# SunJiamei/LRP-ImageCaptioning

Measured on AMD Instinct MI355X. Metric: LRP heatmaps/sec (per predicted token) VGG16+adaptive-attn, 224x224, higher is better.
Workload: dtype bf16x3; 1 GPU; batch=32 synthetic 224x224 per GPU, VGG16 + adaptive-attention, LRP per-token heat-maps, 10 words/caption, V=10000 (BASELINE configs[1]); parallelism=image-sharded x1, RCCL weight broadcast, reverse_walk_precision=bf16x3, handles_per_gpu=2

## Files before the change

### lrp-imagecaptioning_amd/csrc/cnn_kernels.h

```cpp
#pragma once
#include <hip/hip_runtime.h>
#include "conv_igemm.h"

namespace lrp {

__device__ __forceinline__ float safe_den(float z) { return z + (z == 0.f ? 1e-7f : 0.f); }

__global__ __launch_bounds__(256) void im2col_image_kernel(const float* __restrict__ img, float* __restrict__ A1,
                                                           int NB, int H, int W) {
  const size_t idx = (size_t)blockIdx.x * 256 + threadIdx.x;
  const size_t total = (size_t)NB * H * W * 8;
  if (idx >= total) return;
  const int g = (int)(idx & 7);
  const size_t m = idx >> 3;
  const int HW = H * W;
  const int n = (int)(m / HW), rem = (int)(m - (size_t)n * HW);
  const int h = rem / W, w = rem - h * W;
  const bool neg = g >= 4;
  float v[8];
#pragma unroll
  for (int q = 0; q < 8; ++q) {
    const int kk = 8 * (g & 3) + q;
    float x = 0.f;
    if (kk < 27) {
// ... 430 lines not shown
}

__global__ __launch_bounds__(256) void top_divide_split_kernel(const float* __restrict__ R, const float* __restrict__ Ztop,
                                                               const int* __restrict__ row2img, float* __restrict__ S,
                                                               int n, size_t per_img8) {
  const size_t total = (size_t)n * per_img8;
  for (size_t i = (size_t)blockIdx.x * 256 + threadIdx.x; i < total; i += (size_t)gridDim.x * 256) {
    const int t = (int)(i / per_img8);
    const size_t e = i - (size_t)t * per_img8;
    const int img = row2img ? row2img[t] : t;
    const float* r = R + i * 8;
    const float* z = Ztop + ((size_t)img * per_img8 + e) * 8;
    float o[8];
#pragma unroll
    for (int c = 0; c < 8; ++c) o[c] = r[c] / safe_den(z[c]);
    split8_store(o, S + i * 8);
  }
}

constexpr int IMG_T_COLS = 54;
__global__ __launch_bounds__(256) void img_stencil_kernel(const float* __restrict__ T, const float* __restrict__ ximg,
                                                          const int* __restrict__ row2img, float* __restrict__ out,
                                                          int n, int H, int W, int mode) {
  const size_t total = (size_t)n * H * W;
  for (size_t i = (size_t)blockIdx.x * 256 + threadIdx.x; i < total; i += (size_t)gridDim.x * 256) {
    const int HW = H * W;
    const int t = (int)(i / HW), pix = (int)(i - (size_t)t * HW);
    const int h = pix / W, w = pix - h * W;
    float pos[3] = {0.f, 0.f, 0.f}, neg[3] = {0.f, 0.f, 0.f};
#pragma unroll
// ... 81 lines not shown
```

### lrp-imagecaptioning_amd/csrc/decoder.h

```cpp
#pragma once
#include <algorithm>
#include <functional>
#include <map>
#include <string>
#include <vector>

#include "cnn_kernels.h"
#include "common.h"
#include "conv_igemm.h"
#include "decoder_gridtd_kernels.h"
#include "decoder_batched_kernels.h"
#include "decoder_kernels.h"
#include "gradient_kernels.h"
#include "train_gemm.h"

namespace lrp {

struct StateBuf {
  DevBuf buf;
  size_t elem_bytes = 4;
};

struct Decoder {
  int kind = 0, L = 0, D = 0, H = 0, E = 0, V = 0, Tm = 0, B_max = 0, NT_max = 0, sos = 2, eos = 1;
// ... 5 lines not shown
  DevBuf xh, u, att_pre;
  DevBuf state_arena;
  std::map<std::string, StateBuf> state;
  DevBuf cap_dev;
  std::vector<int> cap_host, len_host;
  int* cap_pinned = nullptr;
  hipEvent_t ev_cap = nullptr;
  ~Decoder() {
    if (ev_cap) { (void)hipEventSynchronize(ev_cap); (void)hipEventDestroy(ev_cap); }
    if (cap_pinned) (void)hipHostFree(cap_pinned);
    if (ev_gen) { (void)hipEventSynchronize(ev_gen); (void)hipEventDestroy(ev_gen); }
    if (gen_pinned) (void)hipHostFree(gen_pinned);
  }
  int B_cur = 0;
  bool have_forward = false;
  DevBuf rctx, ravg, tailA, w_ifT_pk;
  DevBuf Wcat2, bcat2, xh1d, xh2d, zg1d, zg2d, hprojd, sprojd, h2u, rho;
  bool bx_ready = false;
  DevBuf bxWg1, bxWg2, bx_rc, bx_rh, bx_rglob, bx_q32, bx_acc32;
  DevBuf bx_g[7];
  bool grad_ready = false;
  DevBuf gW1, gW2, gWglob, gWif, g_seed, g_dc1, g_dc2, g_dg, g_out1, g_out2, g_dglob, g_dwords, g_dctx, g_davg, g_tailA;

  int init(const lrp_config& c, int64_t* total) {
    kind = c.decoder; L = c.L; D = c.D; H = c.H; E = c.E; V = c.V; Tm = c.max_caption_len;
    B_max = c.max_images; NT_max = c.max_tokens; sos = c.sos_id; eos = c.eos_id;
    if (L < 1 || D < 4 || H < 4 || E < 4 || V < 2) return fail(LRP_ERR_INVALID, "bad decoder dims");
    if (D % 8 || H % 8) return fail(LRP_ERR_UNSUPPORTED, "D and H must be multiples of 8");
    if (2 * E + 2 * H > 2048) return fail(LRP_ERR_UNSUPPORTED, "2E+2H too large for the LRP scan (bx_* / gbx_* kernels)");
    const size_t B = B_max, S = Tm + 1;
    struct Want { std::string nm; size_t bytes, eb; };
    std::vector<Want> wants;
    auto st = [&](const char* nm, size_t elems, size_t eb) -> int {
      wants.push_back({nm, elems * eb, eb});
      return LRP_OK;
    };
    if (kind == LRP_DEC_ADAPTIVE) {
      for (const char* nm : {"ht", "ct", "gt", "it_act", "ft_act", "st", "ot_act"}) LRP_TRY(st(nm, B * S * H, 4));
      LRP_TRY(st("attention", B * S * L, 4));
      LRP_TRY(st("beta", B * S, 4));
      LRP_TRY(st("context", B * S * H, 8));
      LRP_TRY(st("c_hat", B * S * H, 8));
      LRP_TRY(st("xt", B * Tm * 2 * E, 4));
      LRP_TRY(st("caption_preds", B * Tm * V, 8));
// ... 14 lines not shown
      LRP_TRY(hprojd.alloc(B * H * 8 * KS_PROJ, total));
      LRP_TRY(sprojd.alloc(B * H * 8 * KS_PROJ, total));
      LRP_TRY(st("#h2u", B * Tm * H, 8));
      LRP_TRY(rho.alloc((size_t)NT_max * Tm * H * 8, total));
    }
    LRP_TRY(vfeat.alloc(B * L * H * 4, total));
    LRP_TRY(if_pre.alloc(B * L * H * 4, total));
    if (kind == LRP_DEC_ADAPTIVE) LRP_TRY(ipre.alloc(B * L * H * 8, total));
    LRP_TRY(stat.alloc(B * L * H * 4, total));
    LRP_TRY(avg.alloc(B * D * 4, total));
    LRP_TRY(glob_pre.alloc(B * E * 4, total));
    LRP_TRY(xh.alloc(B * (2 * E + 2 * H) * 4, total));
    LRP_TRY(att_pre.alloc(B * (L + 1) * 4, total));
    LRP_TRY(st("#u", B * Tm * H, 8));
    {
      size_t off = 0;
      for (const Want& w : wants) off += (w.bytes + 255) / 256 * 256;
      LRP_TRY(state_arena.alloc(off, total));
      off = 0;
      for (const Want& w : wants) {
        if (w.nm == "#u") u.view_of(state_arena, off, w.bytes);
        else if (w.nm == "#h2u") h2u.view_of(state_arena, off, w.bytes);
        else {
          StateBuf& s = state[w.nm];
          s.elem_bytes = w.eb;
          s.buf.view_of(state_arena, off, w.bytes);
        }
        off += (w.bytes + 255) / 256 * 256;
      }
    }
    LRP_TRY(cap_dev.alloc(B * Tm * sizeof(int), total));
    LRP_TRY(rctx.alloc((size_t)NT_max * H * 8, total));
    LRP_TRY(tailA.alloc((size_t)NT_max * L * H * 4, total));
    LRP_TRY(ravg.alloc((size_t)NT_max * D * 8, total));
    cap_host.assign(B * Tm, eos);
    len_host.assign(B, 0);
    return LRP_OK;
  }

  int on_new_features(int B) {
    B_cur = B;
    have_forward = false;
    return LRP_OK;
  }
// ... 29 lines not shown
    LRP_TRY(weight_set_common(nm, ndim, shape, &n));
    DevBuf& d = raw_dev[nm];
    if (d.bytes != n * sizeof(float)) LRP_TRY(d.alloc(n * sizeof(float), total));
    LRP_HIP_CHECK(hipMemcpyAsync(d.p, data, n * sizeof(float), kind, st));
    return LRP_OK;
  }

  static void tr2d(hipStream_t st, const float* src, int lds, int rows, int cols, float* dst, int ldd) {
    hipLaunchKernelGGL(dec_transpose_kernel, dim3((cols + 31) / 32, (rows + 31) / 32), dim3(32, 8), 0, st, src, lds, rows, cols, dst, ldd);
  }
  static hipError_t cp2d(hipStream_t st, const float* src, int lds, int rows, int cols, float* dst, int ldd) {
    return hipMemcpy2DAsync(dst, (size_t)ldd * 4, src, (size_t)lds * 4, (size_t)cols * 4, rows, hipMemcpyDeviceToDevice, st);
  }
  int refresh_from_device(const std::function<const float*(const char*)>& Wd, hipStream_t st) {
    int64_t dummy = 0;
    LRP_TRY(finalize(&dummy, st));
    if (!raw_stale) {
      LRP_TRY(bx_prepare(&dummy, st));
      if (!((H | E | D) & 3)) LRP_TRY(grad_prepare(&dummy, st));
    }
    LRP_TRY(repack_device(Wd, st));
    raw_stale = true;
    return LRP_OK;
  }
  int repack_device(const std::function<const float*(const char*)>& Wd, hipStream_t st) {
    const bool td = kind == LRP_DEC_GRIDTD;
    const float *Wif = Wd("image_features_W"), *Wgl = Wd("global_W");
    const int KD = conv_cinp(D), KH = conv_cinp(H), K4 = conv_cinp(4 * H);
    tr2d(st, Wif, H, D, H, w_if_dual.as<float>(), KD);
    tr2d(st, Wif, H, D, H, w_if_dual.as<float>() + (size_t)H * KD, KD);
// ... 57 lines not shown
    while (want.size() > 1 && want.back() == 1) want.pop_back();
    if (got != want) return fail(LRP_ERR_INVALID, "decoder weight '%s' has the wrong shape", nm);
    return LRP_OK;
  }

  std::function<const float*(const char*)> raw_dev_lookup() {
    return [this](const char* nm) -> const float* { return raw_dev.at(nm).as<float>(); };
  }
  static int zalloc(DevBuf& d, size_t floats, int64_t* total, hipStream_t st) {
    LRP_TRY(d.alloc(floats * sizeof(float), total));
    LRP_HIP_CHECK(hipMemsetAsync(d.p, 0, d.bytes, st));
    return LRP_OK;
  }
  int finalize(int64_t* total, hipStream_t st = nullptr) {
    if (finalized) return LRP_OK;
    const bool td = kind == LRP_DEC_GRIDTD;
    const int K1 = td ? H + 2 * E : 2 * E;
    LRP_TRY(need("image_features_W", {D, H})); LRP_TRY(need("image_features_b", {H}));
    LRP_TRY(need("global_W", {D, E})); LRP_TRY(need("global_b", {E}));
    LRP_TRY(need("embedding", {V, E})); LRP_TRY(need("output_W", {H, V})); LRP_TRY(need("output_b", {V}));
    if (td) {
      LRP_TRY(need("td_Wi", {K1, 4 * H})); LRP_TRY(need("td_Wh", {H, 4 * H})); LRP_TRY(need("td_b", {4 * H}));
      LRP_TRY(need("lang_Wi", {2 * H, 4 * H})); LRP_TRY(need("lang_Wh", {H, 4 * H})); LRP_TRY(need("lang_b", {4 * H}));
      LRP_TRY(need("W_va", {H, H})); LRP_TRY(need("W_ha", {H, H})); LRP_TRY(need("W_a", {H})); LRP_TRY(need("W_x", {K1, H}));
      LRP_TRY(need("W_h", {H, H})); LRP_TRY(need("W_s", {H, H}));
    } else {
      LRP_TRY(need("lstm_Wi", {K1, 4 * H})); LRP_TRY(need("lstm_Wh", {H, 4 * H})); LRP_TRY(need("lstm_b", {4 * H}));
      LRP_TRY(need("Wv", {H, H})); LRP_TRY(need("Wg", {H, H})); LRP_TRY(need("V", {H}));
      LRP_TRY(need("Wx", {K1, H})); LRP_TRY(need("Wh", {H, H})); LRP_TRY(need("Ws", {H, H}));
    }
// ... 55 lines not shown
    if (!cap_pinned) {
      LRP_HIP_CHECK(hipHostMalloc(reinterpret_cast<void**>(&cap_pinned), (size_t)B_max * Tm * sizeof(int)));
      LRP_HIP_CHECK(hipEventCreateWithFlags(&ev_cap, hipEventDisableTiming));
    } else {
      LRP_HIP_CHECK(hipEventSynchronize(ev_cap));
    }
    for (int b = 0; b < B; ++b) {
      len_host[b] = lens[b];
      for (int i = 0; i < Tm; ++i) cap_pinned[b * Tm + i] = cap_host[b * Tm + i] = i < lens[b] ? caps[b * Tm + i] : eos;
    }
    LRP_HIP_CHECK(hipMemcpyAsync(cap_dev.p, cap_pinned, (size_t)B * Tm * sizeof(int), hipMemcpyHostToDevice, st));
    LRP_HIP_CHECK(hipEventRecord(ev_cap, st));
    LRP_TRY(prepare_static(feat_dev, B, st));
    if (kind == LRP_DEC_GRIDTD) return forward_gridtd_steps(B, Tmax, st);
    for (int i = 0; i < Tmax; ++i) LRP_TRY(step_adaptive(i, B, st));
    LRP_HIP_CHECK((skinny<double, double, double>(u.as<double>(), H, Wout.as<float>(), V, bout.as<float>(),
                                                  S_<double>("caption_preds"), V, B * Tm, H, V, 0, st)));
    B_cur = B;
    have_forward = true;
    return LRP_OK;
  }

  int prepare_static(const float* feat_dev, int B, hipStream_t st) {
    LRP_HIP_CHECK(hipMemsetAsync(state_arena.p, 0, state_arena.bytes, st));
    {
      ConvArgs ca{};
      ca.in = feat_dev; ca.NB = B * L; ca.H = 1; ca.W = 1; ca.Cin = D; ca.CinP = conv_cinp(D); ca.taps = 1;
      ca.wpk = w_if_dual.as<float>(); ca.N = 2 * H; ca.split = H; ca.bias = b_if.as<float>();
      ca.out = vfeat.as<float>(); ca.out2 = if_pre.as<float>();
      LRP_HIP_CHECK(conv_launch(EPI_FWD_DUAL, ca, st));
      ConvArgs cv{};
      cv.in = vfeat.as<float>(); cv.NB = B * L; cv.H = 1; cv.W = 1; cv.Cin = H; cv.CinP = conv_cinp(H); cv.taps = 1;
      cv.wpk = w_v.as<float>(); cv.N = H; cv.bias = zero_bias.as<float>(); cv.out = stat.as<float>();
      LRP_HIP_CHECK(conv_launch(EPI_BIAS, cv, st));
    }
    if (kind == LRP_DEC_ADAPTIVE) {
      const size_t ne = (size_t)B * L * H;
      hipLaunchKernelGGL(dec_ipre_kernel, dim3((unsigned)std::min<size_t>((ne + 255) / 256, 2048)), dim3(256), 0, st,
                         if_pre.as<float>(), ipre.as<double>(), ne);
// ... 97 lines not shown
        LRP_TRY(gen_reparent<float>("ct", B, s, st));
      } else {
        for (const char* nm : {"h1t", "c1t", "h2t", "c2t"}) LRP_TRY(gen_reparent<double>(nm, B, s, st));
      }
      hipLaunchKernelGGL(gen_set_word_kernel, dim3((B + 255) / 256), dim3(256), 0, st, cap_dev.as<int>(), gen_idx.as<int>() + B, s, Tm, B);
      LRP_HIP_CHECK(hipGetLastError());
    }
    LRP_TRY(kind == LRP_DEC_ADAPTIVE ? step_adaptive(s, B, st) : step_gridtd(s, B, st));
    const double* rows = (kind == LRP_DEC_ADAPTIVE ? u.as<double>() : h2u.as<double>()) + (size_t)s * H;
    LRP_HIP_CHECK((skinny<double, double, double>(rows, Tm * H, Wout.as<float>(), V, bout.as<float>(), logits_dev, V, B, H, V, 0, st)));
    return LRP_OK;
  }

  int forward_gridtd_steps(int B, int Tmax, hipStream_t st) {
    for (int i = 0; i < Tmax; ++i) LRP_TRY(step_gridtd(i, B, st));
    LRP_HIP_CHECK((skinny<double, double, double>(h2u.as<double>(), H, Wout.as<float>(), V, bout.as<float>(),
                                                  S_<double>("caption_preds"), V, B * Tm, H, V, 0, st)));
    B_cur = B;
    have_forward = true;
    return LRP_OK;
  }
  int step_gridtd(int i, int B, hipStream_t st) {
    const int S = Tm + 1, K1 = H + 2 * E;
    double *h1 = S_<double>("h1t"), *h2 = S_<double>("h2t"), *stt = S_<double>("st");
    {
      hipLaunchKernelGGL(gtd_prep_x1_kernel, dim3(B), dim3(256), 0, st, emb.as<float>(), glob_pre.as<float>(), h1, h2,
                         cap_dev.as<int>(), xh1d.as<double>(), S_<double>("x1t"), i, Tm, E, H, V, sos);
      LRP_HIP_CHECK(hipGetLastError());
      const size_t zs1 = (size_t)B_max * 5 * H, zs2 = (size_t)B_max * 4 * H, ps = (size_t)B_max * H;
      LRP_HIP_CHECK((skinny<double, double, double>(xh1d.as<double>(), K1 + H, Wcat.as<float>(), 5 * H, bcat.as<float>(),
                                                    zg1d.as<double>(), 5 * H, B, K1 + H, 5 * H, 0, st, KS_GATE, zs1)));
      hipLaunchKernelGGL(gtd_pointwise_kernel, dim3(B), dim3(256), 0, st, zg1d.as<double>(), 5 * H, KS_GATE, zs1, h1, S_<double>("c1t"),
// ... 15 lines not shown
                         stat.as<float>(), vvec.as<float>(), if_pre.as<float>(), h1, h2, stt, S_<double>("attention"),
                         S_<double>("beta"), S_<double>("context"), S_<double>("context_hat"), xh2d.as<double>(),
                         S_<double>("x2t"), i, Tm, L, H);
      LRP_HIP_CHECK(hipGetLastError());
      LRP_HIP_CHECK((skinny<double, double, double>(xh2d.as<double>(), 3 * H, Wcat2.as<float>(), 4 * H, bcat2.as<float>(),
                                                    zg2d.as<double>(), 4 * H, B, 3 * H, 4 * H, 0, st, KS_GATE, zs2)));
      hipLaunchKernelGGL(gtd_pointwise_kernel, dim3(B), dim3(256), 0, st, zg2d.as<double>(), 4 * H, KS_GATE, zs2, h2, S_<double>("c2t"),
                         S_<double>("g2t"), S_<double>("i2t_act"), S_<double>("f2t_act"), (double*)nullptr,
                         h2u.as<double>(), S_<double>("o2t_act"), i, Tm, H);
      LRP_HIP_CHECK(hipGetLastError());
    }
    return LRP_OK;
  }

  int explain_gridtd(int n, const int* img_dev, const int* t_dev, const int32_t* t_host, const float* feat_dev,
                     float* R_feat_dev, float* att_dev, double* rwords_dev, hipStream_t st) {
    int64_t dummy = 0;
    LRP_TRY(bx_prepare(&dummy, st));
    int t_max = 0;
    for (int i = 0; i < n; ++i) t_max = std::max(t_max, (int)t_host[i]);
    GbxArgs x{};
    x.img_idx = img_dev; x.tpos = t_dev; x.cap = cap_dev.as<int>();
    x.h1t = S_<double>("h1t"); x.c1t = S_<double>("c1t"); x.g1t = S_<double>("g1t"); x.i1t = S_<double>("i1t_act");
    x.f1t = S_<double>("f1t_act"); x.h2t = S_<double>("h2t"); x.c2t = S_<double>("c2t"); x.g2t = S_<double>("g2t");
    x.i2t = S_<double>("i2t_act"); x.f2t = S_<double>("f2t_act"); x.x1t = S_<double>("x1t"); x.x2t = S_<double>("x2t");
    x.ctx = S_<double>("context"); x.st = S_<double>("st"); x.chat = S_<double>("context_hat"); x.beta = S_<double>("beta");
    x.att = S_<double>("attention"); x.preds = S_<double>("caption_preds");
    x.Wout = Wout.as<float>(); x.WglobT = WglobT.as<float>(); x.avg = avg.as<float>(); x.glob_pre = glob_pre.as<float>();
    x.rc1 = bx_g[0].as<double>(); x.rc2 = bx_g[1].as<double>(); x.rh1 = bx_g[2].as<double>(); x.rh2 = bx_g[3].as<double>();
    x.rchat = bx_g[4].as<double>(); x.nh1 = bx_g[5].as<double>(); x.nh2 = bx_g[6].as<double>();
    x.rglob = bx_rglob.as<double>(); x.q32 = bx_q32.as<float>(); x.acc32 = bx_acc32.as<float>();
    x.rho = rho.as<double>(); x.ravg = ravg.as<double>(); x.att_out = att_dev; x.rwords_out = rwords_dev;
    x.Tm = Tm; x.L = L; x.D = D; x.H = H; x.E = E; x.V = V;
    hipLaunchKernelGGL(gbx_head_kernel, dim3(n), dim3(256), 0, st, x);
    LRP_HIP_CHECK(hipGetLastError());
    for (int s = 0; s < t_max; ++s) {
      hipLaunchKernelGGL(gbx_pre2_kernel, dim3(n), dim3(256), 0, st, x, s);
      LRP_HIP_CHECK(hipGetLastError());
      LRP_TRY(gemm_nt(bx_q32.as<float>(), n, H, bxWg2, 3 * H, bx_acc32.as<float>(), st));
      hipLaunchKernelGGL(gbx_mid_kernel, dim3(n), dim3(256), 0, st, x, s);
      LRP_HIP_CHECK(hipGetLastError());
      LRP_TRY(gemm_nt(bx_q32.as<float>(), n, H, bxWg1, 2 * H + 2 * E, bx_acc32.as<float>(), st));
      hipLaunchKernelGGL(gbx_post_kernel, dim3(n), dim3(256), 0, st, x, s);
      LRP_HIP_CHECK(hipGetLastError());
    }
    hipLaunchKernelGGL(gbx_tail_kernel, dim3(n, (D + 63) / 64), dim3(64), (size_t)E * sizeof(double), st, x);
    LRP_HIP_CHECK(hipGetLastError());
    hipLaunchKernelGGL(gtd_tail_a_kernel, dim3((L * (H / 8) + 255) / 256, n), dim3(256), 0, st, img_dev, t_dev,
                       if_pre.as<float>(), x.att, x.rho, tailA.as<float>(), Tm, L, H);
    LRP_HIP_CHECK(hipGetLastError());
    return tail_gemm(n, img_dev, feat_dev, R_feat_dev, st);
  }

  int grad_prepare(int64_t* total, hipStream_t st = nullptr) {
    if (grad_ready) return LRP_OK;
    if ((H & 3) || (E & 3) || (D & 3)) return fail(LRP_ERR_UNSUPPORTED, "gradient path: H, E, D must be multiples of 4");
    const size_t NT = NT_max;
    if (kind == LRP_DEC_ADAPTIVE) {
      LRP_TRY(pack_alloc_device(gW1, H + 2 * E, 4 * H, total, st));
      LRP_TRY(g_out1.alloc(NT * (H + 2 * E) * 4, total));
    } else {
      LRP_TRY(pack_alloc_device(gW1, 2 * H + 2 * E, 4 * H, total, st));
      LRP_TRY(pack_alloc_device(gW2, 3 * H, 4 * H, total, st));
      LRP_TRY(g_out1.alloc(NT * (2 * H + 2 * E) * 4, total));
      LRP_TRY(g_out2.alloc(NT * 3 * H * 4, total));
      LRP_TRY(g_dc2.alloc(NT * H * 4, total));
// ... 102 lines not shown
    } else {
      LRP_TRY(pack_alloc_device(bxWg1, 2 * H + 2 * E, H, total, st));
      LRP_TRY(pack_alloc_device(bxWg2, 3 * H, H, total, st));
      LRP_TRY(bx_acc32.alloc(NT * (size_t)std::max(2 * H + 2 * E, 3 * H) * 4, total));
      for (DevBuf& d : bx_g) LRP_TRY(d.alloc(NT * H * 8, total));
    }
    LRP_TRY(bx_rc.alloc(NT * H * 8, total));
    LRP_TRY(bx_rh.alloc(NT * H * 8, total));
    LRP_TRY(bx_rglob.alloc(NT * E * 8, total));
    LRP_TRY(bx_q32.alloc(NT * H * 4, total));
    bx_ready = true;
    if (finalized) LRP_TRY(repack_device(raw_dev_lookup(), st));
    return LRP_OK;
  }

  int tail_gemm(int n, const int* img_dev, const float* feat_dev, float* R_feat_dev, hipStream_t st) {
    ConvArgs cg{};
    cg.in = tailA.as<float>(); cg.NB = n; cg.H = L; cg.W = 1; cg.Cin = H; cg.CinP = conv_cinp(H); cg.taps = 1;
    cg.wpk = w_ifT_pk.as<float>(); cg.N = D; cg.aux = feat_dev; cg.row2img = img_dev;
    cg.out = R_feat_dev; cg.out_plain = 1;
    LRP_HIP_CHECK(conv_launch(EPI_MUL, cg, st, PREC_FP32));
    hipLaunchKernelGGL(tail_finish_kernel, dim3((L * D + 255) / 256 > 64 ? 64 : (L * D + 255) / 256, n), dim3(256), 0, st,
                       img_dev, feat_dev, avg.as<float>(), ravg.as<double>(), R_feat_dev, L, D);
    LRP_HIP_CHECK(hipGetLastError());
    return LRP_OK;
  }

  int explain(int n, const int* img_dev, const int* t_dev, const int32_t*, const int32_t* t_host, int variant,
              const float* feat_dev, float* R_feat_dev, float* att_dev, double* rwords_dev, hipStream_t st) {
    if (variant != LRP_EXPLAIN_SEQUENCE && variant != LRP_EXPLAIN_SINGLE_STEP) return fail(LRP_ERR_INVALID, "bad variant");
    if (kind == LRP_DEC_GRIDTD) {
      if (variant != LRP_EXPLAIN_SEQUENCE)
        return fail(LRP_ERR_UNSUPPORTED, "the grid-TD decoder has no single-step variant");
      return explain_gridtd(n, img_dev, t_dev, t_host, feat_dev, R_feat_dev, att_dev, rwords_dev, st);
    }
    int64_t dummy = 0;
    LRP_TRY(bx_prepare(&dummy, st));
    int t_max = 0;
    for (int i = 0; i < n; ++i) t_max = std::max(t_max, (int)t_host[i]);
    BxArgs x{};
    x.img_idx = img_dev; x.tpos = t_dev; x.cap = cap_dev.as<int>();
    x.ht = S_<float>("ht"); x.ct = S_<float>("ct"); x.gt = S_<float>("gt"); x.it = S_<float>("it_act");
    x.ft = S_<float>("ft_act"); x.st = S_<float>("st"); x.beta = S_<float>("beta"); x.att = S_<float>("attention");
    x.xt = S_<float>("xt"); x.ctx = S_<double>("context"); x.chat = S_<double>("c_hat"); x.preds = S_<double>("caption_preds");
    x.Wout = Wout.as<float>(); x.WglobT = WglobT.as<float>(); x.avg = avg.as<float>(); x.glob_pre = glob_pre.as<float>();
    x.rc = bx_rc.as<double>(); x.rh = bx_rh.as<double>(); x.rglob = bx_rglob.as<double>(); x.q32 = bx_q32.as<float>();
    x.acc32 = bx_acc32.as<float>(); x.rctx = rctx.as<double>(); x.ravg = ravg.as<double>(); x.att_out = att_dev;
    x.rwords_out = rwords_dev;
    x.Tm = Tm; x.L = L; x.D = D; x.H = H; x.E = E; x.V = V; x.single_step = variant == LRP_EXPLAIN_SINGLE_STEP;
    hipLaunchKernelGGL(bx_head_kernel, dim3(n), dim3(256), 0, st, x);
    LRP_HIP_CHECK(hipGetLastError());
    const int steps = x.single_step ? 1 : t_max;
    hipLaunchKernelGGL(bx_pre_kernel, dim3(n), dim3(256), 0, st, x, 0);
    LRP_HIP_CHECK(hipGetLastError());
    for (int s = 0; s < steps; ++s) {
      LRP_TRY(gemm_nt(bx_q32.as<float>(), n, H, bxWg1, 2 * E + H, bx_acc32.as<float>(), st));
      hipLaunchKernelGGL(bx_post_kernel, dim3(n), dim3(256), 0, st, x, s, s + 1 < steps ? 1 : 0);
      LRP_HIP_CHECK(hipGetLastError());
    }
    hipLaunchKernelGGL(bx_tail_kernel, dim3(n, (D + 63) / 64), dim3(64), (size_t)E * sizeof(double), st, x);
    LRP_HIP_CHECK(hipGetLastError());
    TailAArgs aa{};
    aa.img_idx = img_dev; aa.tpos = t_dev; aa.vfeat = vfeat.as<float>(); aa.ipre = ipre.as<double>(); aa.att = x.att;
    aa.rho = x.rctx; aa.A = tailA.as<float>(); aa.Tm = Tm; aa.L = L; aa.H = H;
    hipLaunchKernelGGL(tail_a_kernel, dim3((L * (H / 8) + 255) / 256, n), dim3(256), 0, st, aa);
    LRP_HIP_CHECK(hipGetLastError());
    return tail_gemm(n, img_dev, feat_dev, R_feat_dev, st);
  }

  int read_state(const char* name, void* out_dev, size_t out_bytes, hipStream_t st) {
    std::string nm(name);
    const DevBuf* src = nullptr;
    auto it = state.find(nm);
    if (it != state.end()) src = &it->second.buf;
    else if (nm == "image_features_before_act") src = &if_pre;
    else if (nm == "average_img_feature") src = &avg;
    else if (nm == "global_img_feature_before_act") src = &glob_pre;
    else if (nm == "total_static_img_feature" || nm == "image_features_proj") src = &stat;
    if (!src) return fail(LRP_ERR_INVALID, "unknown state array '%s'", name);
    if (out_bytes > src->bytes) return fail(LRP_ERR_INVALID, "state '%s' holds %zu bytes, %zu requested", name, src->bytes, out_bytes);
    LRP_HIP_CHECK(hipMemcpyAsync(out_dev, src->p, out_bytes, hipMemcpyDeviceToDevice, st));
    return LRP_OK;
  }
};

}
```

### lrp-imagecaptioning_amd/csrc/decoder_batched_kernels.h

```cpp
#pragma once
#include "decoder_kernels.h"

namespace lrp {

struct BxArgs {
  const int* img_idx; const int* tpos; const int* cap;
  const float *ht, *ct, *gt, *it, *ft, *st, *beta, *att, *xt;
  const double *ctx, *chat, *preds;
  const float* Wout; const float* WglobT; const float *avg, *glob_pre;
  double *rc, *rh, *rglob;
  float* q32;
  const float* acc32;
  double *rctx, *ravg;
  float* att_out; double* rwords_out;
  int Tm, L, D, H, E, V, single_step;
};

__global__ __launch_bounds__(256) void bx_head_kernel(BxArgs a) {
  const int H = a.H, E = a.E, Tm = a.Tm, S = Tm + 1;
  const int n = blockIdx.x, tid = threadIdx.x;
  const int b = a.img_idx[n], t = a.tpos[n];
  const size_t rowt = (size_t)b * S + t;
  const int k = a.cap[b * Tm + t - 1] - 1;
  const double zk = a.preds[((size_t)b * Tm + (t - 1)) * a.V + k];
  const double bt32_1m = (double)(1.f - a.beta[rowt]);
  const float btf = a.beta[rowt];
  for (int j = tid; j < H; j += 256) {
    const double h = (double)a.ht[rowt * H + j], ch = a.chat[rowt * H + j];
    const double u = h + ch;
    const double r_u = ((double)a.Wout[(size_t)j * a.V + k] * u) / stab(zk) * zk;
    const double su = stab(u);
    const double r_h = h / su * r_u;
    const double r_ch = ch / su * r_u;
    const double sch = stab(ch);
    const double r_ctx = (bt32_1m * a.ctx[rowt * H + j]) / sch * r_ch;
    const double r_s = (double)(btf * a.st[rowt * H + j]) / sch * r_ch;
    a.rctx[(size_t)n * H + j] = r_ctx / stab(a.ctx[rowt * H + j]);
    a.rc[(size_t)n * H + j] = r_s;
    a.rh[(size_t)n * H + j] = r_h;
  }
  for (int e = tid; e < E; e += 256) a.rglob[(size_t)n * E + e] = 0.0;
  if (a.att_out)
    for (int l = tid; l < a.L; l += 256) a.att_out[(size_t)n * a.L + l] = a.att[rowt * a.L + l];
  if (a.rwords_out)
    for (int i = tid; i < Tm; i += 256) a.rwords_out[(size_t)n * Tm + i] = 0.0;
// ... 76 lines not shown
  __syncthreads();
  bx_tail_column(a.WglobT, q, a.avg + (size_t)b * D, a.ravg + (size_t)n * D, blockIdx.y * 64 + tid, E, D);
  if (a.rwords_out && !a.single_step && tid == 0 && blockIdx.y == 0) {
    double* rw = a.rwords_out + (size_t)n * Tm;
    rw[0] = 0.0;
    double m = 0.0;
    for (int i = 0; i < t; ++i) m = fmax(m, fabs(rw[i]));
    for (int i = 0; i + 1 < t; ++i) rw[i] = m != 0.0 ? rw[i + 1] / m : rw[i + 1];
    rw[t - 1] = 0.0;
  }
}

struct GbxArgs {
  const int* img_idx; const int* tpos; const int* cap;
  const double *h1t, *c1t, *g1t, *i1t, *f1t, *h2t, *c2t, *g2t, *i2t, *f2t, *x1t, *x2t;
  const double *ctx, *st, *chat, *beta, *att, *preds;
  const float* Wout; const float* WglobT; const float *avg, *glob_pre;
  double *rc1, *rc2, *rh1, *rh2, *rchat, *nh1, *nh2, *rglob;
  float* q32; const float* acc32;
  double *rho, *ravg;
  float* att_out; double* rwords_out;
  int Tm, L, D, H, E, V;
};

__global__ __launch_bounds__(256) void gbx_head_kernel(GbxArgs a) {
  const int H = a.H, E = a.E, Tm = a.Tm, S = Tm + 1;
  const int n = blockIdx.x, tid = threadIdx.x;
  const int b = a.img_idx[n], t = a.tpos[n];
  const size_t rowt = (size_t)b * S + t, o = (size_t)n * H;
  const int k = a.cap[b * Tm + t - 1] - 1;
  const double zk = a.preds[((size_t)b * Tm + (t - 1)) * a.V + k];
  for (int j = tid; j < H; j += 256) {
    const double h2 = a.h2t[rowt * H + j], ch = a.chat[rowt * H + j];
    const double u = h2 + ch;
    const double r_u = ((double)a.Wout[(size_t)j * a.V + k] * u) / stab(zk) * zk;
    a.rh2[o + j] = h2 / stab(u) * r_u;
    a.rchat[o + j] = ch / stab(u) * r_u;
    a.rc1[o + j] = 0.0; a.rc2[o + j] = 0.0; a.rh1[o + j] = 0.0;
  }
  for (int e = tid; e < E; e += 256) a.rglob[(size_t)n * E + e] = 0.0;
  if (a.att_out)
    for (int l = tid; l < a.L; l += 256) a.att_out[(size_t)n * a.L + l] = (float)a.att[rowt * a.L + l];
  if (a.rwords_out)
    for (int i = tid; i < Tm; i += 256) a.rwords_out[(size_t)n * Tm + i] = 0.0;
}

__global__ __launch_bounds__(256) void gbx_pre2_kernel(GbxArgs a, int s) {
  const int H = a.H, S = a.Tm + 1;
  const int n = blockIdx.x, tid = threadIdx.x;
  const int b = a.img_idx[n], i = a.tpos[n] - 1 - s;
// ... 82 lines not shown
```

### lrp-imagecaptioning_amd/csrc/encoder.h

```cpp
#pragma once
#include <algorithm>
#include <functional>
#include <memory>
#include <string>
#include <vector>

#include "cnn_kernels.h"
#include "common.h"
#include "conv_igemm.h"
#include "conv_sparse.h"
#include "f16_operand.h"

namespace lrp {

struct ConvLayer {
  std::string name;
  int cin = 0, cout = 0, H = 0, W = 0;
  bool pool_after = false;
  bool have_w = false, have_b = false;
  DevBuf w_fwd;
  DevBuf w_fwd_a;
  DevBuf w_fwd_zs;
  DevBuf w_fwd_as;
  DevBuf w_fwd_h;
// ... 34 lines not shown
  int top_h = 0, top_w = 0, top_c = 0;
  std::vector<ConvLayer> layers;
  DevBuf images;
  DevBuf a1;
  DevBuf bufX, bufA, bufZ;
  DevBuf bufXs;
  DevBuf bufXl;
  DevBuf feat;
  DevBuf ztop;
  DevBuf s0, s1;
  int encoded = 0;
  bool features_only = false;
  bool profile = false;
  int prec = PREC_BF16X3;
  const int* row2img_host = nullptr;
  bool walk_f16 = false;
  int64_t t2_mask_user = -1;
  bool two_term(int li) const {
    if (li <= 0 || li >= (int)layers.size()) return false;
    if (t2_mask_user >= 0) return ((t2_mask_user >> li) & 1) != 0;
    int last_pool = -1;
    for (size_t q = 0; q < layers.size(); ++q)
      if (layers[q].pool_after) last_pool = (int)q;
    return li <= last_pool && 9 * layers[li].cout >= 576 && 9 * layers[li].cin >= 576;
  }
  DevBuf sp_scp;
  DevBuf act_max, act_unscale;
  DevBuf out_scale;
  static bool fwd_emit() { return sw().fwd_emit != 0; }
  DevBuf tok_exp, tok_max, tok_fac;
// ... 514 lines not shown
  }

  int full_gate(int li, hipStream_t st) {
    ConvLayer& L = layers[li];
    if (!L.pool_after || L.gfull_epoch == encode_epoch) return LRP_OK;
    if (!L.Gc.p || L.gc_epoch != encode_epoch) return fail(LRP_ERR_STATE, "no pool gate of layer %d for this encode", li);
    const size_t n8 = (size_t)encoded * (L.H / 2) * (L.W / 2) * (L.cout / 8);
    hipLaunchKernelGGL(pool_gate_expand_kernel, dim3(stream_grid(n8)), dim3(256), 0, st, L.Gc.as<float>(), L.Gpos.as<unsigned char>(),
                       L.G.as<float>(), encoded, L.H, L.W, L.cout);
    LRP_HIP_CHECK(hipGetLastError());
    L.gfull_epoch = encode_epoch;
    return LRP_OK;
  }

  int explain(int n, const int* row2img_dev, const float* R_feat_dev, float* R_img_dev, hipStream_t st, int walk = 0,
              const std::function<int(int, const float*)>* layer_hook = nullptr) {
    const int* r2i_host = row2img_host;
    row2img_host = nullptr;
    if (n < 1 || n > max_tokens) return fail(LRP_ERR_INVALID, "n=%d outside [1,%d]", n, max_tokens);
    if (walk < 0 || walk > 3) return fail(LRP_ERR_INVALID, "unknown walk %d", walk);
    if (encoded < 1 || features_only) return fail(LRP_ERR_STATE, "lrp_encode_images must run before the CNN explain");
    if (gates_pending) LRP_HIP_CHECK(hipStreamWaitEvent(st, ev_gates, 0));
    const ConvLayer& T = layers.back();
    float* S = s0.as<float>();
    float* Snext = s1.as<float>();
    bool split = prec == PREC_BF16X3 && walk == 0;
    bool hook_split = prec == PREC_BF16X3 && walk == 1 && layer_hook != nullptr;
    for (const ConvLayer& L : layers)
      if (L.cout & 7) split = hook_split = false;
    for (size_t li = 1; li < layers.size(); ++li)
      if (!layers[li].w_bwd_full_s.p) hook_split = false;
    const bool f16 = split && walk_f16 && img_fused();
    if (f16) {
// ... 10 lines not shown
    auto lev_max = [&](int lev) { return tok_max.as<unsigned>() + (size_t)lev * max_tokens; };
    const int run_prec = f16 ? PREC_F16X2 : (split || hook_split) ? PREC_BF16X3 : PREC_FP32;
    if (walk != 0) {
      const size_t per4 = T.act_elems() / 4;
      hipLaunchKernelGGL(grad_top_kernel, dim3(stream_grid((size_t)n * per4)), dim3(256), 0, st,
                         reinterpret_cast<const f32x4*>(R_feat_dev), feat.as<f32x4>(), row2img_dev,
                         reinterpret_cast<f32x4*>(S), n, per4, walk == 3 ? 1 : 0);
      LRP_HIP_CHECK(hipGetLastError());
    } else if (f16) {
      const int top = (int)layers.size() - 1;
      hipLaunchKernelGGL(top_divide_f16_kernel, dim3(n), dim3(256), 0, st, R_feat_dev, ztop.as<float>(), row2img_dev, S,
                         T.act_elems() / 8, lev_exp(top), lev_max(top));
      LRP_HIP_CHECK(hipGetLastError());
    } else if (split) {
      const size_t per8 = T.act_elems() / 8;
      hipLaunchKernelGGL(top_divide_split_kernel, dim3(stream_grid((size_t)n * per8)), dim3(256), 0, st, R_feat_dev,
                         ztop.as<float>(), row2img_dev, S, n, per8);
      LRP_HIP_CHECK(hipGetLastError());
    } else {
      const size_t per4 = T.act_elems() / 4;
      hipLaunchKernelGGL(top_divide_kernel, dim3(stream_grid((size_t)n * per4)), dim3(256), 0, st,
                         reinterpret_cast<const f32x4*>(R_feat_dev), ztop.as<f32x4>(), row2img_dev,
                         reinterpret_cast<f32x4*>(S), n, per4);
      LRP_HIP_CHECK(hipGetLastError());
    }
    const bool up2_on = sw().up2_compact != 0;
    bool pairs_in = false;
    const bool fold_on = sw().img_fold != 0 && split && !f16 && walk == 0 && !layer_hook && img_fused() && layers.size() > 1 &&
                         !layers[0].pool_after && layers[1].cin == 64 && layers[0].w_bwd_s.p != nullptr;
    auto walk_plan = [&](int lc, bool up2) {
      const ConvLayer& Lc = layers[lc];
      ConvAsk q;
// ... 164 lines not shown
```

### lrp-imagecaptioning_amd/csrc/engine.hip

```cpp
#include <hip/hip_runtime.h>

#include <cmath>
#include <cstring>
#include <exception>
#include <map>
#include <new>
#include <string>
#include <vector>

#include "common.h"
#include "conv_igemm.h"
#include "conv_sparse.h"
#include "decoder.h"
#include "encoder.h"
#include "eval_kernels.h"
#include "gradcam_kernels.h"
#include "resnet_encoder.h"
#include "rules_kernels.h"
#include "score_kernels.h"
#include "trainer.h"

namespace lrp {
std::string& last_error_ref() {
  static thread_local std::string e;
// ... 285 lines not shown
    if (!h || !img_idx_host || !R_feat_dev || !R_img_dev) return fail(LRP_ERR_INVALID, "null argument");
    if (h->encoded() < 1 || h->features_only()) return fail(LRP_ERR_STATE, "lrp_encode_images must run before lrp_cnn_explain");
    LRP_TRY(stage_indices(h, n, img_idx_host, nullptr, false, S(stream)));
    if (h->resnet) return h->rn.explain(n, h->idx_dev.as<int>(), R_feat_dev, R_img_dev, S(stream));
    h->enc.row2img_host = h->idx_pinned;
    return h->enc.explain(n, h->idx_dev.as<int>(), R_feat_dev, R_img_dev, S(stream));
  });
}

int lrp_explain_tokens(lrp_handle* h, int32_t n, const int32_t* img_idx_host, const int32_t* t_host, int32_t variant,
                       float* R_img_dev, float* R_feat_dev, float* att_dev, double* r_words_dev, void* stream) {
  return with_handle(h, [&]() -> int {
    if (!h || !img_idx_host || !t_host || !R_img_dev) return fail(LRP_ERR_INVALID, "null argument");
    LRP_TRY(stage_indices(h, n, img_idx_host, t_host, true, S(stream)));
    float* rf = R_feat_dev ? R_feat_dev : h->rfeat_tmp.as<float>();
    LRP_TRY(h->dec.explain(n, h->idx_dev.as<int>(), h->idx_dev.as<int>() + n, img_idx_host, t_host, variant,
                           h->feat(), rf, att_dev, r_words_dev, S(stream)));
    if (h->resnet) return h->rn.explain(n, h->idx_dev.as<int>(), rf, R_img_dev, S(stream));
    h->enc.row2img_host = h->idx_pinned;
    return h->enc.explain(n, h->idx_dev.as<int>(), rf, R_img_dev, S(stream));
  });
}

int lrp_decoder_gradient(lrp_handle* h, int32_t n, const int32_t* img_idx_host, const int32_t* t_host, float* d_feat_dev,
                         double* r_words_dev, void* stream) {
  return with_handle(h, [&]() -> int {
    if (!h || !img_idx_host || !t_host || !d_feat_dev) return fail(LRP_ERR_INVALID, "null argument");
    if (h->cfg.decoder == LRP_DEC_ADAPTIVE && h->cfg.E != h->cfg.H)
      return fail(LRP_ERR_UNSUPPORTED, "the adaptive gradient baseline needs E == H (E=%d, H=%d): the reference's class cannot run there "
                                       "(explainers.py:798 sizes d_xt E + H wide, :823 stores a 2E-wide row into it and raises), so "
                                       "no reference defines the result",
                  h->cfg.E, h->cfg.H);
    LRP_TRY(stage_indices(h, n, img_idx_host, t_host, true, S(stream)));
    int t_max = 0;
    for (int i = 0; i < n; ++i) t_max = t_host[i] > t_max ? t_host[i] : t_max;
// ... 555 lines not shown
```

Before: 10290 heatmaps/s.

## Defer vocabulary logits to on-demand and fuse tail finish into CNN top divide

The forward pass no longer computes the full B*Tm x V caption_preds GEMM. Logits are marked stale and materialised lazily only when they are read or finalized, and the LRP scan kernels recompute the single needed logit with a small in-block dot product over u and a Wout column. The caption_preds region is moved to the end of the state arena so the per-forward memset can skip it. Separately, when the CNN head uses split bf16, the decoder's tail_finish pass is folded into the encoder's top divide-and-split kernel, removing one full pass over R_feat. This adds complexity to the state tracking and uses strided Wout column reads inside the scan.

```diff
diff --git a/lrp-imagecaptioning_amd/csrc/cnn_kernels.h b/lrp-imagecaptioning_amd/csrc/cnn_kernels.h
--- a/lrp-imagecaptioning_amd/csrc/cnn_kernels.h
+++ b/lrp-imagecaptioning_amd/csrc/cnn_kernels.h
@@ -1,6 +1,7 @@
 #pragma once
 #include <hip/hip_runtime.h>
 #include "conv_igemm.h"
+#include "decoder_kernels.h"
 
 namespace lrp {
 
@@ -468,6 +469,33 @@
     float o[8];
 #pragma unroll
     for (int c = 0; c < 8; ++c) o[c] = r[c] / safe_den(z[c]);
+    split8_store(o, S + i * 8);
+  }
+}
+
+__global__ __launch_bounds__(256) void tail_finish_divide_split_kernel(const float* __restrict__ R, const float* __restrict__ F,
+                                                                       const float* __restrict__ avg, const double* __restrict__ ravg,
+                                                                       const float* __restrict__ Ztop, const int* __restrict__ row2img,
+                                                                       float* __restrict__ S, int n, int L, int D) {
+  const size_t per_img8 = (size_t)L * D / 8, total = (size_t)n * per_img8;
+  for (size_t i = (size_t)blockIdx.x * 256 + threadIdx.x; i < total; i += (size_t)gridDim.x * 256) {
+    const int t = (int)(i / per_img8);
+    const size_t e = i - (size_t)t * per_img8;
+    const int img = row2img ? row2img[t] : t;
+    const int d0 = (int)((e * 8) % D);
+    const float* r = R + i * 8;
+    const float* f = F + ((size_t)img * per_img8 + e) * 8;
+    const float* z = Ztop + ((size_t)img * per_img8 + e) * 8;
+    const float* av = avg + (size_t)img * D + d0;
+    const double* ra = ravg + (size_t)t * D + d0;
+    float o[8];
+#pragma unroll
+    for (int c = 0; c < 8; ++c) {
+      const float fl = f[c] / (float)L;
+      const float first = (float)((double)fl / stab((double)av[c]) * ra[c]);
+      const float rf = (float)((double)first + (double)r[c]);
+      o[c] = rf / safe_den(z[c]);
+    }
     split8_store(o, S + i * 8);
   }
 }
diff --git a/lrp-imagecaptioning_amd/csrc/decoder.h b/lrp-imagecaptioning_amd/csrc/decoder.h
--- a/lrp-imagecaptioning_amd/csrc/decoder.h
+++ b/lrp-imagecaptioning_amd/csrc/decoder.h
@@ -43,6 +43,9 @@
   }
   int B_cur = 0;
   bool have_forward = false;
+  enum { PREDS_VALID = 0, PREDS_STALE = 1, PREDS_ZERO = 2 };
+  int preds_state = PREDS_ZERO, preds_rows = 0;
+  size_t arena_zero_bytes = 0;
   DevBuf rctx, ravg, tailA, w_ifT_pk;
   DevBuf Wcat2, bcat2, xh1d, xh2d, zg1d, zg2d, hprojd, sprojd, h2u, rho;
   bool bx_ready = false;
@@ -56,7 +59,7 @@
     B_max = c.max_images; NT_max = c.max_tokens; sos = c.sos_id; eos = c.eos_id;
     if (L < 1 || D < 4 || H < 4 || E < 4 || V < 2) return fail(LRP_ERR_INVALID, "bad decoder dims");
     if (D % 8 || H % 8) return fail(LRP_ERR_UNSUPPORTED, "D and H must be multiples of 8");
-    if (2 * E + 2 * H > 2048) return fail(LRP_ERR_UNSUPPORTED, "2E+2H too large for the LRP scan (bx_* / gbx_* kernels)");
+    if (2 * E + 2 * H > BX_SCAN_MAX) return fail(LRP_ERR_UNSUPPORTED, "2E+2H too large for the LRP scan (bx_* / gbx_* kernels)");
     const size_t B = B_max, S = Tm + 1;
     struct Want { std::string nm; size_t bytes, eb; };
     std::vector<Want> wants;
@@ -101,11 +104,13 @@
     LRP_TRY(att_pre.alloc(B * (L + 1) * 4, total));
     LRP_TRY(st("#u", B * Tm * H, 8));
     {
+      std::stable_partition(wants.begin(), wants.end(), [](const Want& w) { return w.nm != "caption_preds"; });
       size_t off = 0;
       for (const Want& w : wants) off += (w.bytes + 255) / 256 * 256;
       LRP_TRY(state_arena.alloc(off, total));
       off = 0;
       for (const Want& w : wants) {
+        if (w.nm == "caption_preds") arena_zero_bytes = off;
         if (w.nm == "#u") u.view_of(state_arena, off, w.bytes);
         else if (w.nm == "#h2u") h2u.view_of(state_arena, off, w.bytes);
         else {
@@ -115,6 +120,7 @@
         }
         off += (w.bytes + 255) / 256 * 256;
       }
+      if (!state.count("caption_preds")) arena_zero_bytes = off;
     }
     LRP_TRY(cap_dev.alloc(B * Tm * sizeof(int), total));
     LRP_TRY(rctx.alloc((size_t)NT_max * H * 8, total));
@@ -174,6 +180,7 @@
   }
   int refresh_from_device(const std::function<const float*(const char*)>& Wd, hipStream_t st) {
     int64_t dummy = 0;
+    LRP_TRY(materialise_preds(st));
     LRP_TRY(finalize(&dummy, st));
     if (!raw_stale) {
       LRP_TRY(bx_prepare(&dummy, st));
@@ -261,6 +268,7 @@
   }
   int finalize(int64_t* total, hipStream_t st = nullptr) {
     if (finalized) return LRP_OK;
+    LRP_TRY(materialise_preds(st));
     const bool td = kind == LRP_DEC_GRIDTD;
     const int K1 = td ? H + 2 * E : 2 * E;
     LRP_TRY(need("image_features_W", {D, H})); LRP_TRY(need("image_features_b", {H}));
@@ -346,15 +354,27 @@
     LRP_TRY(prepare_static(feat_dev, B, st));
     if (kind == LRP_DEC_GRIDTD) return forward_gridtd_steps(B, Tmax, st);
     for (int i = 0; i < Tmax; ++i) LRP_TRY(step_adaptive(i, B, st));
-    LRP_HIP_CHECK((skinny<double, double, double>(u.as<double>(), H, Wout.as<float>(), V, bout.as<float>(),
-                                                  S_<double>("caption_preds"), V, B * Tm, H, V, 0, st)));
+    preds_state = PREDS_STALE;
+    preds_rows = B * Tm;
     B_cur = B;
     have_forward = true;
     return LRP_OK;
   }
 
+  int materialise_preds(hipStream_t st) {
+    if (preds_state == PREDS_VALID) return LRP_OK;
+    StateBuf& p = state["caption_preds"];
+    LRP_HIP_CHECK(hipMemsetAsync(p.buf.p, 0, p.buf.bytes, st));
+    if (preds_state == PREDS_STALE)
+      LRP_HIP_CHECK((skinny<double, double, double>((kind == LRP_DEC_GRIDTD ? h2u : u).as<double>(), H, Wout.as<float>(), V,
+                                                    bout.as<float>(), p.buf.as<double>(), V, preds_rows, H, V, 0, st)));
+    preds_state = PREDS_VALID;
+    return LRP_OK;
+  }
+
   int prepare_static(const float* feat_dev, int B, hipStream_t st) {
-    LRP_HIP_CHECK(hipMemsetAsync(state_arena.p, 0, state_arena.bytes, st));
+    LRP_HIP_CHECK(hipMemsetAsync(state_arena.p, 0, arena_zero_bytes, st));
+    preds_state = PREDS_ZERO;
     {
       ConvArgs ca{};
       ca.in = feat_dev; ca.NB = B * L; ca.H = 1; ca.W = 1; ca.Cin = D; ca.CinP = conv_cinp(D); ca.taps = 1;
@@ -482,8 +502,8 @@
 
   int forward_gridtd_steps(int B, int Tmax, hipStream_t st) {
     for (int i = 0; i < Tmax; ++i) LRP_TRY(step_gridtd(i, B, st));
-    LRP_HIP_CHECK((skinny<double, double, double>(h2u.as<double>(), H, Wout.as<float>(), V, bout.as<float>(),
-                                                  S_<double>("caption_preds"), V, B * Tm, H, V, 0, st)));
+    preds_state = PREDS_STALE;
+    preds_rows = B * Tm;
     B_cur = B;
     have_forward = true;
     return LRP_OK;
@@ -529,7 +549,7 @@
   }
 
   int explain_gridtd(int n, const int* img_dev, const int* t_dev, const int32_t* t_host, const float* feat_dev,
-                     float* R_feat_dev, float* att_dev, double* rwords_dev, hipStream_t st) {
+                     float* R_feat_dev, float* att_dev, double* rwords_dev, hipStream_t st, bool defer_finish = false) {
     int64_t dummy = 0;
     LRP_TRY(bx_prepare(&dummy, st));
     int t_max = 0;
@@ -540,8 +560,8 @@
     x.f1t = S_<double>("f1t_act"); x.h2t = S_<double>("h2t"); x.c2t = S_<double>("c2t"); x.g2t = S_<double>("g2t");
     x.i2t = S_<double>("i2t_act"); x.f2t = S_<double>("f2t_act"); x.x1t = S_<double>("x1t"); x.x2t = S_<double>("x2t");
     x.ctx = S_<double>("context"); x.st = S_<double>("st"); x.chat = S_<double>("context_hat"); x.beta = S_<double>("beta");
-    x.att = S_<double>("attention"); x.preds = S_<double>("caption_preds");
-    x.Wout = Wout.as<float>(); x.WglobT = WglobT.as<float>(); x.avg = avg.as<float>(); x.glob_pre = glob_pre.as<float>();
+    x.att = S_<double>("attention"); x.h2u = h2u.as<double>();
+    x.Wout = Wout.as<float>(); x.bout = bout.as<float>(); x.WglobT = WglobT.as<float>(); x.avg = avg.as<float>(); x.glob_pre = glob_pre.as<float>();
     x.rc1 = bx_g[0].as<double>(); x.rc2 = bx_g[1].as<double>(); x.rh1 = bx_g[2].as<double>(); x.rh2 = bx_g[3].as<double>();
     x.rchat = bx_g[4].as<double>(); x.nh1 = bx_g[5].as<double>(); x.nh2 = bx_g[6].as<double>();
     x.rglob = bx_rglob.as<double>(); x.q32 = bx_q32.as<float>(); x.acc32 = bx_acc32.as<float>();
@@ -564,7 +584,7 @@
     hipLaunchKernelGGL(gtd_tail_a_kernel, dim3((L * (H / 8) + 255) / 256, n), dim3(256), 0, st, img_dev, t_dev,
                        if_pre.as<float>(), x.att, x.rho, tailA.as<float>(), Tm, L, H);
     LRP_HIP_CHECK(hipGetLastError());
-    return tail_gemm(n, img_dev, feat_dev, R_feat_dev, st);
+    return tail_gemm(n, img_dev, feat_dev, R_feat_dev, st, defer_finish);
   }
 
   int grad_prepare(int64_t* total, hipStream_t st = nullptr) {
@@ -697,12 +717,13 @@
     return LRP_OK;
   }
 
-  int tail_gemm(int n, const int* img_dev, const float* feat_dev, float* R_feat_dev, hipStream_t st) {
+  int tail_gemm(int n, const int* img_dev, const float* feat_dev, float* R_feat_dev, hipStream_t st, bool defer_finish = false) {
     ConvArgs cg{};
     cg.in = tailA.as<float>(); cg.NB = n; cg.H = L; cg.W = 1; cg.Cin = H; cg.CinP = conv_cinp(H); cg.taps = 1;
     cg.wpk = w_ifT_pk.as<float>(); cg.N = D; cg.aux = feat_dev; cg.row2img = img_dev;
     cg.out = R_feat_dev; cg.out_plain = 1;
     LRP_HIP_CHECK(conv_launch(EPI_MUL, cg, st, PREC_FP32));
+    if (defer_finish) return LRP_OK;
     hipLaunchKernelGGL(tail_finish_kernel, dim3((L * D + 255) / 256 > 64 ? 64 : (L * D + 255) / 256, n), dim3(256), 0, st,
                        img_dev, feat_dev, avg.as<float>(), ravg.as<double>(), R_feat_dev, L, D);
     LRP_HIP_CHECK(hipGetLastError());
@@ -710,12 +731,13 @@
   }
 
   int explain(int n, const int* img_dev, const int* t_dev, const int32_t*, const int32_t* t_host, int variant,
-              const float* feat_dev, float* R_feat_dev, float* att_dev, double* rwords_dev, hipStream_t st) {
+              const float* feat_dev, float* R_feat_dev, float* att_dev, double* rwords_dev, hipStream_t st,
+              bool defer_finish = false) {
     if (variant != LRP_EXPLAIN_SEQUENCE && variant != LRP_EXPLAIN_SINGLE_STEP) return fail(LRP_ERR_INVALID, "bad variant");
     if (kind == LRP_DEC_GRIDTD) {
       if (variant != LRP_EXPLAIN_SEQUENCE)
         return fail(LRP_ERR_UNSUPPORTED, "the grid-TD decoder has no single-step variant");
-      return explain_gridtd(n, img_dev, t_dev, t_host, feat_dev, R_feat_dev, att_dev, rwords_dev, st);
+      return explain_gridtd(n, img_dev, t_dev, t_host, feat_dev, R_feat_dev, att_dev, rwords_dev, st, defer_finish);
     }
     int64_t dummy = 0;
     LRP_TRY(bx_prepare(&dummy, st));
@@ -725,8 +747,8 @@
     x.img_idx = img_dev; x.tpos = t_dev; x.cap = cap_dev.as<int>();
     x.ht = S_<float>("ht"); x.ct = S_<float>("ct"); x.gt = S_<float>("gt"); x.it = S_<float>("it_act");
     x.ft = S_<float>("ft_act"); x.st = S_<float>("st"); x.beta = S_<float>("beta"); x.att = S_<float>("attention");
-    x.xt = S_<float>("xt"); x.ctx = S_<double>("context"); x.chat = S_<double>("c_hat"); x.preds = S_<double>("caption_preds");
-    x.Wout = Wout.as<float>(); x.WglobT = WglobT.as<float>(); x.avg = avg.as<float>(); x.glob_pre = glob_pre.as<float>();
+    x.xt = S_<float>("xt"); x.ctx = S_<double>("context"); x.chat = S_<double>("c_hat"); x.u = u.as<double>();
+    x.Wout = Wout.as<float>(); x.bout = bout.as<float>(); x.WglobT = WglobT.as<float>(); x.avg = avg.as<float>(); x.glob_pre = glob_pre.as<float>();
     x.rc = bx_rc.as<double>(); x.rh = bx_rh.as<double>(); x.rglob = bx_rglob.as<double>(); x.q32 = bx_q32.as<float>();
     x.acc32 = bx_acc32.as<float>(); x.rctx = rctx.as<double>(); x.ravg = ravg.as<double>(); x.att_out = att_dev;
     x.rwords_out = rwords_dev;
@@ -748,7 +770,7 @@
     aa.rho = x.rctx; aa.A = tailA.as<float>(); aa.Tm = Tm; aa.L = L; aa.H = H;
     hipLaunchKernelGGL(tail_a_kernel, dim3((L * (H / 8) + 255) / 256, n), dim3(256), 0, st, aa);
     LRP_HIP_CHECK(hipGetLastError());
-    return tail_gemm(n, img_dev, feat_dev, R_feat_dev, st);
+    return tail_gemm(n, img_dev, feat_dev, R_feat_dev, st, defer_finish);
   }
 
   int read_state(const char* name, void* out_dev, size_t out_bytes, hipStream_t st) {
@@ -761,6 +783,7 @@
     else if (nm == "global_img_feature_before_act") src = &glob_pre;
     else if (nm == "total_static_img_feature" || nm == "image_features_proj") src = &stat;
     if (!src) return fail(LRP_ERR_INVALID, "unknown state array '%s'", name);
+    if (nm == "caption_preds") LRP_TRY(materialise_preds(st));
     if (out_bytes > src->bytes) return fail(LRP_ERR_INVALID, "state '%s' holds %zu bytes, %zu requested", name, src->bytes, out_bytes);
     LRP_HIP_CHECK(hipMemcpyAsync(out_dev, src->p, out_bytes, hipMemcpyDeviceToDevice, st));
     return LRP_OK;
diff --git a/lrp-imagecaptioning_amd/csrc/decoder_batched_kernels.h b/lrp-imagecaptioning_amd/csrc/decoder_batched_kernels.h
--- a/lrp-imagecaptioning_amd/csrc/decoder_batched_kernels.h
+++ b/lrp-imagecaptioning_amd/csrc/decoder_batched_kernels.h
@@ -2,12 +2,40 @@
 #include "decoder_kernels.h"
 
 namespace lrp {
+
+constexpr int BX_SCAN_MAX = 2048;
+constexpr int BX_HMAX = 1024;
+static_assert(BX_SCAN_MAX / 2 <= BX_HMAX, "bx_logit stages H <= (BX_SCAN_MAX - 2E) / 2 values");
+__device__ __forceinline__ double bx_logit(const double* __restrict__ u_row, const float* __restrict__ Wout,
+                                           const float* __restrict__ bout, int H, int V, int k, const float** wcol) {
+  __shared__ double s_u[BX_HMAX];
+  __shared__ float s_w[BX_HMAX];
+  __shared__ double s_part[4];
+  const int tid = threadIdx.x;
+  for (int j = tid; j < H; j += 256) { s_u[j] = u_row[j]; s_w[j] = Wout[(size_t)j * V + k]; }
+  __syncthreads();
+  if ((tid & 63) == 0) {
+    const int kg = tid >> 6;
+    double acc = 0.0;
+    for (int k0 = 0; k0 < H; k0 += 64) {
+#pragma unroll
+      for (int kk = 0; kk < 16; ++kk) {
+        const int j = k0 + kg * 16 + kk;
+        if (j < H) acc = fma(s_u[j], (double)s_w[j], acc);
+      }
+    }
+    s_part[kg] = acc;
+  }
+  __syncthreads();
+  *wcol = s_w;
+  return s_part[0] + s_part[1] + s_part[2] + s_part[3] + (double)bout[k];
+}
 
 struct BxArgs {
   const int* img_idx; const int* tpos; const int* cap;
   const float *ht, *ct, *gt, *it, *ft, *st, *beta, *att, *xt;
-  const double *ctx, *chat, *preds;
-  const float* Wout; const float* WglobT; const float *avg, *glob_pre;
+  const double *ctx, *chat, *u;
+  const float* Wout; const float* bout; const float* WglobT; const float *avg, *glob_pre;
   double *rc, *rh, *rglob;
   float* q32;
   const float* acc32;
@@ -22,13 +50,14 @@
   const int b = a.img_idx[n], t = a.tpos[n];
   const size_t rowt = (size_t)b * S + t;
   const int k = a.cap[b * Tm + t - 1] - 1;
-  const double zk = a.preds[((size_t)b * Tm + (t - 1)) * a.V + k];
+  const float* wk;
+  const double zk = bx_logit(a.u + ((size_t)b * Tm + (t - 1)) * H, a.Wout, a.bout, H, a.V, k, &wk);
   const double bt32_1m = (double)(1.f - a.beta[rowt]);
   const float btf = a.beta[rowt];
   for (int j = tid; j < H; j += 256) {
     const double h = (double)a.ht[rowt * H + j], ch = a.chat[rowt * H + j];
     const double u = h + ch;
-    const double r_u = ((double)a.Wout[(size_t)j * a.V + k] * u) / stab(zk) * zk;
+    const double r_u = ((double)wk[j] * u) / stab(zk) * zk;
     const double su = stab(u);
     const double r_h = h / su * r_u;
     const double r_ch = ch / su * r_u;
@@ -135,8 +164,8 @@
 struct GbxArgs {
   const int* img_idx; const int* tpos; const int* cap;
   const double *h1t, *c1t, *g1t, *i1t, *f1t, *h2t, *c2t, *g2t, *i2t, *f2t, *x1t, *x2t;
-  const double *ctx, *st, *chat, *beta, *att, *preds;
-  const float* Wout; const float* WglobT; const float *avg, *glob_pre;
+  const double *ctx, *st, *chat, *beta, *att, *h2u;
+  const float* Wout; const float* bout; const float* WglobT; const float *avg, *glob_pre;
   double *rc1, *rc2, *rh1, *rh2, *rchat, *nh1, *nh2, *rglob;
   float* q32; const float* acc32;
   double *rho, *ravg;
@@ -150,11 +179,12 @@
   const int b = a.img_idx[n], t = a.tpos[n];
   const size_t rowt = (size_t)b * S + t, o = (size_t)n * H;
   const int k = a.cap[b * Tm + t - 1] - 1;
-  const double zk = a.preds[((size_t)b * Tm + (t - 1)) * a.V + k];
+  const float* wk;
+  const double zk = bx_logit(a.h2u + ((size_t)b * Tm + (t - 1)) * H, a.Wout, a.bout, H, a.V, k, &wk);
   for (int j = tid; j < H; j += 256) {
     const double h2 = a.h2t[rowt * H + j], ch = a.chat[rowt * H + j];
     const double u = h2 + ch;
-    const double r_u = ((double)a.Wout[(size_t)j * a.V + k] * u) / stab(zk) * zk;
+    const double r_u = ((double)wk[j] * u) / stab(zk) * zk;
     a.rh2[o + j] = h2 / stab(u) * r_u;
     a.rchat[o + j] = ch / stab(u) * r_u;
     a.rc1[o + j] = 0.0; a.rc2[o + j] = 0.0; a.rh1[o + j] = 0.0;
diff --git a/lrp-imagecaptioning_amd/csrc/encoder.h b/lrp-imagecaptioning_amd/csrc/encoder.h
--- a/lrp-imagecaptioning_amd/csrc/encoder.h
+++ b/lrp-imagecaptioning_amd/csrc/encoder.h
@@ -72,6 +72,13 @@
   bool profile = false;
   int prec = PREC_BF16X3;
   const int* row2img_host = nullptr;
+  struct TopShare { const float* avg; const double* ravg; int D; };
+  bool head_is_split() const {
+    if (prec != PREC_BF16X3 || (walk_f16 && img_fused())) return false;
+    for (const ConvLayer& L : layers)
+      if (L.cout & 7) return false;
+    return true;
+  }
   bool walk_f16 = false;
   int64_t t2_mask_user = -1;
   bool two_term(int li) const {
@@ -616,9 +623,10 @@
   }
 
   int explain(int n, const int* row2img_dev, const float* R_feat_dev, float* R_img_dev, hipStream_t st, int walk = 0,
-              const std::function<int(int, const float*)>* layer_hook = nullptr) {
+              const std::function<int(int, const float*)>* layer_hook = nullptr, const TopShare* share = nullptr) {
     const int* r2i_host = row2img_host;
     row2img_host = nullptr;
+    if (share && (walk != 0 || !head_is_split())) return fail(LRP_ERR_STATE, "deferred mean-pool share without the split-bf16 head");
     if (n < 1 || n > max_tokens) return fail(LRP_ERR_INVALID, "n=%d outside [1,%d]", n, max_tokens);
     if (walk < 0 || walk > 3) return fail(LRP_ERR_INVALID, "unknown walk %d", walk);
     if (encoded < 1 || features_only) return fail(LRP_ERR_STATE, "lrp_encode_images must run before the CNN explain");
@@ -659,8 +667,13 @@
       LRP_HIP_CHECK(hipGetLastError());
     } else if (split) {
       const size_t per8 = T.act_elems() / 8;
-      hipLaunchKernelGGL(top_divide_split_kernel, dim3(stream_grid((size_t)n * per8)), dim3(256), 0, st, R_feat_dev,
-                         ztop.as<float>(), row2img_dev, S, n, per8);
+      if (share)
+        hipLaunchKernelGGL(tail_finish_divide_split_kernel, dim3(stream_grid((size_t)n * per8)), dim3(256), 0, st, R_feat_dev,
+                           feat.as<float>(), share->avg, share->ravg, ztop.as<float>(), row2img_dev, S, n,
+                           (int)(T.act_elems() / share->D), share->D);
+      else
+        hipLaunchKernelGGL(top_divide_split_kernel, dim3(stream_grid((size_t)n * per8)), dim3(256), 0, st, R_feat_dev,
+                           ztop.as<float>(), row2img_dev, S, n, per8);
       LRP_HIP_CHECK(hipGetLastError());
     } else {
       const size_t per4 = T.act_elems() / 4;
diff --git a/lrp-imagecaptioning_amd/csrc/engine.hip b/lrp-imagecaptioning_amd/csrc/engine.hip
--- a/lrp-imagecaptioning_amd/csrc/engine.hip
+++ b/lrp-imagecaptioning_amd/csrc/engine.hip
@@ -323,11 +323,13 @@
     if (!h || !img_idx_host || !t_host || !R_img_dev) return fail(LRP_ERR_INVALID, "null argument");
     LRP_TRY(stage_indices(h, n, img_idx_host, t_host, true, S(stream)));
     float* rf = R_feat_dev ? R_feat_dev : h->rfeat_tmp.as<float>();
+    const bool one_pass = !R_feat_dev && !h->resnet && h->enc.head_is_split();
     LRP_TRY(h->dec.explain(n, h->idx_dev.as<int>(), h->idx_dev.as<int>() + n, img_idx_host, t_host, variant,
-                           h->feat(), rf, att_dev, r_words_dev, S(stream)));
+                           h->feat(), rf, att_dev, r_words_dev, S(stream), one_pass));
     if (h->resnet) return h->rn.explain(n, h->idx_dev.as<int>(), rf, R_img_dev, S(stream));
+    const Encoder::TopShare share{h->dec.avg.as<float>(), h->dec.ravg.as<double>(), h->cfg.D};
     h->enc.row2img_host = h->idx_pinned;
-    return h->enc.explain(n, h->idx_dev.as<int>(), rf, R_img_dev, S(stream));
+    return h->enc.explain(n, h->idx_dev.as<int>(), rf, R_img_dev, S(stream), 0, nullptr, one_pass ? &share : nullptr);
   });
 }
 
```

Measured after the change: 10340 heatmaps/s, median of 6. No clear change (+0.5%).
